# Monokaix/etcd

Measured on AMD Instinct MI355X. Metric: quorum group-evals/sec at 1/2/4/8 MI355X; % HBM peak; speedup vs Go host, higher is better.
Workload: dtype u64; 1 GPU; config2_n5: 64M groups x 5-voter MajorityConfig CommittedIndex+VoteResult (TallyVotes counts into the stats); groups_per_gpu=67108864, global_groups=67108864, voters=5

## Files before the change

etcd_amd/csrc/qe_progress.hpp:

```cpp
#pragma once
#include "qe_tile.hpp"

namespace qe {

constexpr int kRingChunk = 8;

template <bool ACCT>
struct Acct {
  uint64_t b = 0;
  __device__ __forceinline__ void add(bool on, uint32_t bytes) {
    if constexpr (ACCT) b += on ? bytes : 0u;
  }
};
template <bool ACCT>
__device__ __forceinline__ void acct_flush(const Acct<ACCT> &ac, uint64_t *acct) {
  if constexpr (ACCT) {
    uint64_t b = ac.b;
#pragma unroll
    for (int d = 32; d >= 1; d >>= 1) b += __shfl_xor(b, d, 64);
    if ((threadIdx.x & 63) == 0 && acct)
      atomicAdd(reinterpret_cast<unsigned long long *>(acct), static_cast<unsigned long long>(b));
  }
}

// ... 103 lines not shown
  uint32_t added = 0;
  if (x.row) {
    uint32_t fit = 1;
    if (x.me) {
      const uint64_t me = x.me;
      uint32_t q = d >= 4 * me ? 4u : 0u;
      q += d >= (q + 2) * me ? 2u : 0u;
      q += d >= (q + 1) * me ? 1u : 0u;
      fit += q;
    }
    added = x.me ? (lim < fit ? lim : fit) : (lim ? 1u : 0u);
    if (added) {
      if (run.n == 0) {
        run.p = ring_pos(p.start, p.count, x.F);
        run.b = p.next;
      }
      run.n += added;
      const PRun here{0, 0, p.next};
      p.next = run_val(here, added - 1, x.me, x.li) + 1;
      p.count += added;
      ac.add(true, x.eb * added);
    }
  } else {
    while (__builtin_amdgcn_ballot_w64(added < lim && p.next <= x.li)) {
      const bool on = added < lim && p.next <= x.li;
      const PRun here{0, 0, p.next};
      const uint64_t last = run_val(here, 0, x.me, x.li);
      const uint32_t pos = ring_pos(p.start, p.count, x.F);
      ring_add_mem<AUX>(p, x, on, pos, last);
      if (on) {
        if (run.n == 0) {
          run.p = pos;
          run.b = p.next;
        }
        run.n += 1;
        p.next = last + 1;
        p.count += 1;
        added += 1;
      }
      ac.add(on, x.eb);
    }
  }
  if (repl) {
    nmsg = added;
    if (!loop && sei && added < k && p.count < x.F && p.next > x.li) nmsg += k - added;
  }
  if (nmsg) {
    if (x.count_msgs == 0) x.first_index = idx0;
    const uint32_t c = x.count_msgs + (nmsg < 255u ? nmsg : 255u);
    x.count_msgs = c < 255u ? c : 255u;
  }
}

template <bool P>
__device__ __forceinline__ void ring_load_n16(const PSend &x, bool ld, uint32_t rep, uint32_t FP,
                                              uint32_t (&lo)[kRingChunk],
                                              uint32_t (&hi)[kRingChunk], const uint32_t *pre,
                                              uint64_t nx_old) {
  u32x4 a = {0, 0, 0, 0};
  if (pre) {
    a = u32x4{pre[0], pre[1], pre[2], pre[3]};
  } else if (__builtin_amdgcn_ballot_w64(ld)) {
    a = bld128(x.r16, ld ? (threadIdx.x & 63) * 16 : kOOB);
  }
  const uint64_t top = nx_old - 1;
  const uint32_t w4[4] = {a.x, a.y, a.z, a.w};
#pragma unroll
  for (int k = 0; k < kRingChunk; k++) {
    const uint64_t e = top - ((w4[k >> 1] >> (16 * (k & 1))) & 0xFFFFu);
    lo[k] = static_cast<uint32_t>(e);
    hi[k] = static_cast<uint32_t>(e >> 32);
  }
  const bool w = ld && rep_wide(rep);
  if (__builtin_amdgcn_ballot_w64(w)) {
    const u32x4 l0 = bld128(x.rlo, w ? x.lb : kOOB);
    const u32x4 h0 = bld128(x.rhi, w ? x.lb : kOOB);
    u32x4 l1 = {0, 0, 0, 0}, h1 = {0, 0, 0, 0};
    if (FP > 4) {
      l1 = bld128(x.rlo, w ? x.lb + 16 : kOOB);
      h1 = bld128(x.rhi, w ? x.lb + 16 : kOOB);
    }
    if constexpr (P)
      asm volatile("" ::"v"(l0.x), "v"(l0.y), "v"(l0.z), "v"(l0.w), "v"(h0.x), "v"(h0.y),
                   "v"(h0.z), "v"(h0.w), "v"(l1.x), "v"(l1.y), "v"(l1.z), "v"(l1.w), "v"(h1.x),
                   "v"(h1.y), "v"(h1.z), "v"(h1.w));
    if (w) {
      lo[0] = l0.x, lo[1] = l0.y, lo[2] = l0.z, lo[3] = l0.w;
      lo[4] = l1.x, lo[5] = l1.y, lo[6] = l1.z, lo[7] = l1.w;
      hi[0] = h0.x, hi[1] = h0.y, hi[2] = h0.z, hi[3] = h0.w;
      hi[4] = h1.x, hi[5] = h1.y, hi[6] = h1.z, hi[7] = h1.w;
    }
  }
}

template <bool P>
__device__ __forceinline__ void ring_load_row(const PSend &x, bool ld, uint32_t rep, uint32_t FP,
                                              uint32_t (&lo)[kRingChunk],
                                              uint32_t (&hi)[kRingChunk],
                                              const uint32_t *pre = nullptr) {
#pragma unroll
  for (int k = 0; k < kRingChunk; k++) lo[k] = (pre && ld) ? pre[k] : 0u;
  if (!pre && __builtin_amdgcn_ballot_w64(ld)) {
    const u32x4 a = bld128(x.rlo, ld ? x.lb : kOOB);
    lo[0] = a.x, lo[1] = a.y, lo[2] = a.z, lo[3] = a.w;
    if (FP > 4) {
      const u32x4 b = bld128(x.rlo, ld ? x.lb + 16 : kOOB);
      lo[4] = b.x, lo[5] = b.y, lo[6] = b.z, lo[7] = b.w;
    }
  }
  const uint32_t ep = rep_epoch(rep);
#pragma unroll
  for (int k = 0; k < kRingChunk; k++) hi[k] = ep;
  const bool w = ld && rep_wide(rep);
  if (__builtin_amdgcn_ballot_w64(w)) {
    const u32x4 a = bld128(x.rhi, w ? x.lb : kOOB);
    u32x4 b = {0, 0, 0, 0};
    if (FP > 4) b = bld128(x.rhi, w ? x.lb + 16 : kOOB);
    if constexpr (P)
      asm volatile("" ::"v"(a.x), "v"(a.y), "v"(a.z), "v"(a.w), "v"(b.x), "v"(b.y), "v"(b.z),
                   "v"(b.w));
    if (w) hi[0] = a.x, hi[1] = a.y, hi[2] = a.z, hi[3] = a.w;
    if (w) hi[4] = b.x, hi[5] = b.y, hi[6] = b.z, hi[7] = b.w;
  }
}

struct RunLo {
  uint32_t lob, lod, jcap;
};
__device__ __forceinline__ RunLo run_lo(const PRun &r, uint32_t me, uint64_t li) {
  const uint64_t d = li - r.b;
  uint32_t q = 0;
  if (me) {
    const uint64_t m = me;
    q = d >= 4 * m ? 4u : 0u;
    q += d >= (q + 2) * m ? 2u : 0u;
    q += d >= (q + 1) * m ? 1u : 0u;
    q = d >= 8 * m ? 8u : q;
  }
  return RunLo{static_cast<uint32_t>(r.b), static_cast<uint32_t>(d), q};
}
__device__ __forceinline__ uint32_t run_lo_at(const RunLo &L, uint32_t j, uint32_t me) {
  return L.lob + (j < L.jcap ? (j + 1) * me - 1u : L.lod);
}

template <bool P>
// ... 19 lines not shown
    if (!__builtin_amdgcn_ballot_w64(wl && !ok)) {
      const RunLo L1 = run_lo(r1, x.me, x.li), L2 = run_lo(r2, x.me, x.li);
#pragma unroll
      for (int k = 0; k < kRingChunk; k++) {
        if (static_cast<uint32_t>(k) >= x.F) break;
        const uint32_t j1 = static_cast<uint32_t>(k) >= r1.p ? k - r1.p : k + x.F - r1.p;
        const uint32_t j2 = static_cast<uint32_t>(k) >= r2.p ? k - r2.p : k + x.F - r2.p;
        lo[k] = j2 < r2.n ? run_lo_at(L2, j2, x.me) : (j1 < r1.n ? run_lo_at(L1, j1, x.me) : lo[k]);
      }
      if (wl) p.rep = p.count ? QE_PW_EPOCH_BITS(h) : 0u;
      if (P || __builtin_amdgcn_ballot_w64(wl)) {
        bst128(u32x4{lo[0], lo[1], lo[2], lo[3]}, x.rlo, wl ? x.lb : kOOB);
        if (FP > 4) bst128(u32x4{lo[4], lo[5], lo[6], lo[7]}, x.rlo, wl ? x.lb + 16 : kOOB);
      }
      return;
    }
  }
  uint32_t h0 = 0;
  bool seen = false, uni = true;
  const uint32_t st = p.start;
#pragma unroll
  for (int k = 0; k < kRingChunk; k++) {
    if (static_cast<uint32_t>(k) >= x.F) break;
    const uint32_t j1 = static_cast<uint32_t>(k) >= r1.p ? k - r1.p : k + x.F - r1.p;
    const uint32_t j2 = static_cast<uint32_t>(k) >= r2.p ? k - r2.p : k + x.F - r2.p;
    const bool on1 = j1 < r1.n, on2 = j2 < r2.n;
    if (on1 || on2) {
      const uint64_t v = on2 ? run_val(r2, j2, x.me, x.li) : run_val(r1, j1, x.me, x.li);
      lo[k] = static_cast<uint32_t>(v);
      hi[k] = static_cast<uint32_t>(v >> 32);
    }
    const uint32_t rel = static_cast<uint32_t>(k) >= st ? k - st : k + x.F - st;
    if (rel < p.count) {
      uni = uni && (!seen || hi[k] == h0);
      h0 = seen ? h0 : hi[k];
      seen = true;
    }
  }
  const bool wide = seen && (!uni || h0 > QE_RING_EPOCH_MAX);
  if (wl) p.rep = !seen ? 0u : (wide ? QE_PF_RING_WIDE : QE_PW_EPOCH_BITS(h0));
  if (__builtin_amdgcn_ballot_w64(wl)) {
    bst128(u32x4{lo[0], lo[1], lo[2], lo[3]}, x.rlo, wl ? x.lb : kOOB);
    if (FP > 4) bst128(u32x4{lo[4], lo[5], lo[6], lo[7]}, x.rlo, wl ? x.lb + 16 : kOOB);
  }
  const bool wh = wl && wide;
  if (__builtin_amdgcn_ballot_w64(wh)) {
    bst128(u32x4{hi[0], hi[1], hi[2], hi[3]}, x.rhi, wh ? x.lb : kOOB);
    if (FP > 4) bst128(u32x4{hi[4], hi[5], hi[6], hi[7]}, x.rhi, wh ? x.lb + 16 : kOOB);
  }
}

template <bool P>
__device__ __forceinline__ void ring_store_n16(PR &p, const PSend &x, const PRun &r1,
                                               const PRun &r2, bool touched, uint64_t nx_old,
                                               uint32_t FP, uint32_t (&lo)[kRingChunk],
                                               uint32_t (&hi)[kRingChunk]) {
  const bool any = (r1.n | r2.n) != 0;
  const bool wl = touched && p.count > 0 && (any || p.next != nx_old);
  if (!P && !__builtin_amdgcn_ballot_w64(wl)) return;
  const uint64_t top = p.next - 1;
  const uint32_t st = p.start;
  bool fits = true;
  uint32_t o[4] = {0, 0, 0, 0};
#pragma unroll
  for (int k = 0; k < kRingChunk; k++) {
    const uint32_t j1 = static_cast<uint32_t>(k) >= r1.p ? k - r1.p : k + x.F - r1.p;
    const uint32_t j2 = static_cast<uint32_t>(k) >= r2.p ? k - r2.p : k + x.F - r2.p;
    const bool on1 = j1 < r1.n, on2 = j2 < r2.n;
    const uint64_t v = on2 ? run_val(r2, j2, x.me, x.li)
                           : (on1 ? run_val(r1, j1, x.me, x.li) : ent64(hi[k], lo[k]));
    lo[k] = static_cast<uint32_t>(v);
    hi[k] = static_cast<uint32_t>(v >> 32);
    const uint32_t rel = static_cast<uint32_t>(k) >= st ? k - st : k + x.F - st;
    const bool live = static_cast<uint32_t>(k) < x.F && rel < p.count;
    fits = fits && (!live || (v <= top && top - v <= 0xFFFFull));
    o[k >> 1] |= (static_cast<uint32_t>(top - v) & 0xFFFFu) << (16 * (k & 1));
  }
  if (wl) p.rep = fits ? 0u : QE_PF_RING_WIDE;
  if (P || __builtin_amdgcn_ballot_w64(wl))
    bst128(u32x4{o[0], o[1], o[2], o[3]}, x.r16, (wl && fits) ? (threadIdx.x & 63) * 16 : kOOB);
  const bool ww = wl && !fits;
  if (__builtin_amdgcn_ballot_w64(ww)) {
    bst128(u32x4{lo[0], lo[1], lo[2], lo[3]}, x.rlo, ww ? x.lb : kOOB);
    bst128(u32x4{hi[0], hi[1], hi[2], hi[3]}, x.rhi, ww ? x.lb : kOOB);
    if (FP > 4) {
      bst128(u32x4{lo[4], lo[5], lo[6], lo[7]}, x.rlo, ww ? x.lb + 16 : kOOB);
      bst128(u32x4{hi[4], hi[5], hi[6], hi[7]}, x.rhi, ww ? x.lb + 16 : kOOB);
    }
  }
}

__device__ __forceinline__ void ring_append_n16(PR &p, const PSend &x, const PRun &run, bool on,
                                                uint64_t nx_old, uint32_t rep_old, u32x4 raw,
                                                uint32_t FP) {
  const bool wl = on && p.count > 0 && (run.n != 0 || p.next != nx_old);
  if (!__builtin_amdgcn_ballot_w64(wl)) return;
  const uint64_t d64 = p.next - nx_old;
  const uint32_t delta = d64 > 0xFFFFull ? 0x10000u : static_cast<uint32_t>(d64);
  const uint32_t w4[4] = {raw.x, raw.y, raw.z, raw.w};
  const uint32_t st = p.start;
  bool fits = !rep_wide(rep_old);
  uint32_t o[4] = {0, 0, 0, 0};
#pragma unroll
  for (int k = 0; k < kRingChunk; k++) {
    const uint32_t j = static_cast<uint32_t>(k) >= run.p ? k - run.p : k + x.F - run.p;
    const uint32_t rel = static_cast<uint32_t>(k) >= st ? k - st : k + x.F - st;
    const bool live = static_cast<uint32_t>(k) < x.F && rel < p.count;
    uint32_t off;
    if (j < run.n) {
      const uint64_t d = p.next - 1 - run_val(run, j, x.me, x.li);
      off = d > 0xFFFFull ? 0x10000u : static_cast<uint32_t>(d);
    } else {
      off = ((w4[k >> 1] >> (16 * (k & 1))) & 0xFFFFu) + delta;
    }
    fits = fits && (!live || off <= 0xFFFFu);
    o[k >> 1] |= (off & 0xFFFFu) << (16 * (k & 1));
  }
  if (wl && fits) p.rep = 0u;
  bst128(u32x4{o[0], o[1], o[2], o[3]}, x.r16, (wl && fits) ? (threadIdx.x & 63) * 16 : kOOB);
  const bool slow = wl && !fits;
  if (__builtin_amdgcn_ballot_w64(slow)) {
    const bool was_wide = rep_wide(rep_old);
    const uint64_t top_old = nx_old - 1;
    const uint64_t vnew = run.n ? run_val(run, 0, x.me, x.li) : 0;
#pragma unroll 1
    for (uint32_t k = 0; k < x.F; k++) {
      const bool isnew = run.n != 0 && k == run.p;
      const bool wr = slow && (isnew || !was_wide);
      const uint32_t h = k >> 1;
      const uint32_t wd = h == 0 ? raw.x : (h == 1 ? raw.y : (h == 2 ? raw.z : raw.w));
      const uint64_t v = isnew ? vnew : top_old - ((wd >> (16 * (k & 1))) & 0xFFFFu);
      bst32(static_cast<uint32_t>(v), x.rlo, wr ? x.lb + k * 4 : kOOB);
      bst32(static_cast<uint32_t>(v >> 32), x.rhi, wr ? x.lb + k * 4 : kOOB);
    }
    if (slow) p.rep = QE_PF_RING_WIDE;
  }
}

template <bool ACCT>
__device__ __forceinline__ void free_le(PR &p, uint64_t to, uint32_t c_old, uint32_t fr_old,
// ... 72 lines not shown
}
template <typename MT>
__device__ __forceinline__ void ovf_st(uint32_t v, rsrc_t r, uint32_t off) {
  if constexpr (sizeof(MT) == 1) __builtin_amdgcn_raw_buffer_store_b8(static_cast<uint8_t>(v), r, off, 0, 0);
  else __builtin_amdgcn_raw_buffer_store_b16(static_cast<uint16_t>(v), r, off, 0, 0);
}
__device__ __forceinline__ void ovf_fence() { asm volatile("s_waitcnt vmcnt(0)" ::: "memory"); }

struct PB {
  uint64_t mt, ix, nx, hn, lt;
  uint32_t w;
  uint32_t rc;
  uint32_t rl[kRingChunk];
};

struct SlotArgs {
  uint64_t stride;
  uint32_t F, FP;
  uint64_t *match, *next, *pending;
  uint32_t *pw, *ilo, *ihi;
  uint16_t *infl16;
  const uint64_t *mhint, *mlogterm;
  const uint32_t *read_ctx;
  uint8_t *msg_count;
  uint64_t *msg_index;
};

template <bool P>
__device__ __forceinline__ SlotArgs slot_args(const PArgs &a) {
  if constexpr (P) {
    typedef const PArgs __attribute__((address_space(4))) KA;
    KA *ka = (KA *)__builtin_amdgcn_kernarg_segment_ptr();
    asm volatile("" : "+s"(ka));
    return SlotArgs{ka->stride, ka->F, ka->FP, ka->match, ka->next, ka->pending, ka->pw,
                    ka->ilo, ka->ihi, ka->infl16, ka->mhint, ka->mlogterm, ka->read_ctx,
                    ka->msg_count, ka->msg_index};
  } else {
    return SlotArgs{a.stride, a.F, a.FP, a.match, a.next, a.pending, a.pw, a.ilo, a.ihi,
                    a.infl16, a.mhint, a.mlogterm, a.read_ctx, a.msg_count, a.msg_index};
  }
}

template <bool P, bool RD, bool N16, class A>
__device__ __forceinline__ void pb_load(const A &a, uint64_t row, const uint64_t *l_mix,
                                        uint32_t n, uint32_t lane, bool ld, bool rej,
                                        bool has_ix, bool rcl, PB &b) {
  b.mt = l_mix[lane];
  b.ix = has_ix ? l_mix[64 + lane] : 0;
  if constexpr (P) {
    const bool rl = ld;
    if constexpr (N16) {
      const u32x4 x0 = bld128(mk_rsrc(a.infl16 + row * QE_RING16_MAX_F, n * 16), rl ? lane * 16 : kOOB);
      b.rl[0] = x0.x, b.rl[1] = x0.y, b.rl[2] = x0.z, b.rl[3] = x0.w;
      b.rl[4] = b.rl[5] = b.rl[6] = b.rl[7] = 0u;
    } else {
      const rsrc_t rr = mk_rsrc(a.ilo + row * a.FP, n * a.FP * 4);
      const uint32_t lb = lane * a.FP * 4;
      const u32x4 x0 = bld128(rr, rl ? lb : kOOB);
      const u32x4 x1 = bld128(rr, (rl && a.FP > 4) ? lb + 16 : kOOB);
      b.rl[0] = x0.x, b.rl[1] = x0.y, b.rl[2] = x0.z, b.rl[3] = x0.w;
      b.rl[4] = x1.x, b.rl[5] = x1.y, b.rl[6] = x1.z, b.rl[7] = x1.w;
    }
    b.nx = bld64(mk_rsrc(a.next + row, n * 8), ld ? lane * 8 : kOOB);
    b.w = bld32(mk_rsrc(a.pw + row, n * 4), ld ? lane * 4 : kOOB);
    b.hn = bld64(mk_rsrc(a.mhint + row, n * 8), rej ? lane * 8 : kOOB);
    b.lt = bld64(mk_rsrc(a.mlogterm + row, n * 8), rej ? lane * 8 : kOOB);
    if constexpr (RD) b.rc = bld32(opt_rsrc(a.read_ctx, row, n), rcl ? lane * 4 : kOOB);
    else b.rc = 0;
    return;
  }
  if (__builtin_amdgcn_ballot_w64(ld)) {
    b.nx = bld64(mk_rsrc(a.next + row, n * 8), ld ? lane * 8 : kOOB);
    b.w = bld32(mk_rsrc(a.pw + row, n * 4), ld ? lane * 4 : kOOB);
  } else {
    b.nx = 0;
    b.w = 0;
  }
  if (__builtin_amdgcn_ballot_w64(rej)) {
    b.hn = bld64(mk_rsrc(a.mhint + row, n * 8), rej ? lane * 8 : kOOB);
    b.lt = bld64(mk_rsrc(a.mlogterm + row, n * 8), rej ? lane * 8 : kOOB);
  } else {
    b.hn = b.lt = 0;
  }
  if (__builtin_amdgcn_ballot_w64(rcl)) b.rc = bld32(mk_rsrc(a.read_ctx + row, n * 4), rcl ? lane * 4 : kOOB);
  else b.rc = 0;
}

template <bool P>
__device__ __forceinline__ void pb_ready(const PB &b) {
  if constexpr (P) return;
  asm volatile("" ::"v"(b.nx), "v"(b.w), "v"(b.hn), "v"(b.lt), "v"(b.rc));
}

#ifndef QE_PSTEP_WAVES
#define QE_PSTEP_WAVES 3
#endif

template <int S, typename MT, bool MASKED, bool JOINT, int RM, bool ACCT, bool RD,
          int WPB = kBlock / 64, bool P = false, bool N16 = false>
__global__ __attribute__((amdgpu_flat_work_group_size(1, 64 * WPB),
                          amdgpu_waves_per_eu(S <= 9 ? ((N16 && P && !RD && S <= 5) ? 4 : QE_PSTEP_WAVES)
                                                     : 2))) void
k_progress_step(PArgs a) {
  constexpr int CH = kRingChunk;
  constexpr uint32_t kFull = (1u << S) - 1u;
  using QT = typename std::conditional<sizeof(MT) == 1, uint32_t, uint64_t>::type;
  constexpr uint32_t EW = 8 * sizeof(MT);
  constexpr uint32_t kRQ = QE_READ_QUEUE;
  constexpr bool OVF = RD;
  uint32_t n_groups = 0, n_adv = 0, n_viol = 0, n_read = 0;
  uint64_t sum_c = 0, csum = 0;
  Acct<ACCT> ac;
  const uint32_t lane = threadIdx.x & 63;
  const uint64_t wave =
      static_cast<uint64_t>(blockIdx.x) * WPB + __builtin_amdgcn_readfirstlane(threadIdx.x >> 6);
  const uint64_t nwaves = static_cast<uint64_t>(gridDim.x) * WPB;
  const uint64_t ntiles = (a.G + 63) / 64;
  const uint32_t F = a.F;
  static_assert(!P || (S <= 9 && !ACCT), "pipelined form: S <= 9, no accounting");
  const bool row_ring = P || F <= CH;
  constexpr int HD = P ? 2 : 0;
  const uint32_t o8 = lane * 8;
  __shared__ uint64_t l_mix[WPB][S][2][64];
  __shared__ uint64_t l_run[WPB][RM][2][64];
  const uint32_t wv = threadIdx.x >> 6;
  for (uint64_t t = wave; t < ntiles; t += nwaves) {
    const uint64_t g0 = t * 64;
    const uint32_t n = tile_n(a.G, t);
    const bool live = lane < n;
    uint32_t nr = 0;
    const uint32_t mi =
        MASKED ? (ld_mask_r<MT>(mk_rsrc(static_cast<const MT *>(a.inc) + g0, n * sizeof(MT)), lane) &
                  kFull)
               : kFull;
    const uint32_t mo =
        JOINT ? (ld_mask_r<MT>(mk_rsrc(static_cast<const MT *>(a.out) + g0, n * sizeof(MT)), lane) &
                 kFull)
              : 0u;
    const uint32_t trk =
        a.tracked ? (ld_mask_r<MT>(mk_rsrc(static_cast<const MT *>(a.tracked) + g0,
                                           n * sizeof(MT)), lane) & kFull)
                  : kFull;
    const uint32_t self = a.self_slot ? bld8(mk_rsrc(a.self_slot + g0, n), lane) : 0xFFu;
    const uint32_t ltr0 = a.transferee ? bld8(mk_rsrc(a.transferee + g0, n), lane) : 0xFFu;
    uint32_t ltr = ltr0;
    const uint64_t li = bld64(mk_rsrc(a.last_index + g0, n * 8), o8);
    const uint64_t fi = bld64(mk_rsrc(a.first_index + g0, n * 8), o8);
    const uint64_t ts = bld64(mk_rsrc(a.term_start + g0, n * 8), o8);
    const rsrc_t r_commit = mk_rsrc(a.committed + g0, n * 8);
    const uint64_t c0 = bld64(r_commit, o8);
    const uint64_t snap_ld = a.snap_index ? bld64(mk_rsrc(a.snap_index + g0, n * 8), o8) : 0;
    const bool rd = RD && a.read_acks != nullptr;
    uint32_t qh = 0, qn = 0;
    QT q0 = 0;
    if (rd) {
      qn = bld8(mk_rsrc(a.read_count + g0, n), lane);
      qn = qn < a.read_cap ? qn : a.read_cap;
      qh = bld32(mk_rsrc(a.read_head + g0, n * 4), o8 >> 1);
      if constexpr (sizeof(QT) == 4)
        q0 = bld32(mk_rsrc(static_cast<const QT *>(a.read_acks) + g0, n * 4), o8 >> 1);
      else
        q0 = bld64(mk_rsrc(static_cast<const QT *>(a.read_acks) + g0, n * 8), o8);
    }
    const uint32_t dctx = qn ? qh + qn - 1u : 0u;
    const uint32_t qn0 = qn;
    QT q = q0;
    bool qtouch = false;
    uint32_t nrel = 0;
    ac.add(live, (MASKED ? sizeof(MT) : 0) + (JOINT ? sizeof(MT) : 0) +
                     (a.tracked ? sizeof(MT) : 0) + (a.self_slot ? 1 : 0) +
                     (a.transferee ? 1 : 0) + 32 + (a.snap_index ? 8 : 0) + (rd ? 5 : 0) +
                     ((rd && qn0) ? sizeof(QT) : 0));
    uint64_t m0[S];
    uint32_t ty[S];
    uint64_t ix[S];
#pragma unroll
    for (int s = 0; s < S; s++) {
      const uint64_t row = static_cast<uint64_t>(s) * a.stride + g0;
      const bool tr = (trk >> s) & 1u;
      m0[s] = bld64(mk_rsrc(a.match + row, n * 8), o8);
      ty[s] = bld8(mk_rsrc(a.mtype + row, n), tr ? lane : kOOB);
// ... 9 lines not shown
      for (int r = 0; r < RM; r++) {
        const uint64_t rrow = static_cast<uint64_t>(r) * a.stride + g0;
        const uint32_t off = static_cast<uint32_t>(r) < a.R ? o8 : kOOB;
        rr0[r] = bld64(mk_rsrc(a.run_first + rrow, n * 8), off);
        rr1[r] = bld64(mk_rsrc(a.run_term + rrow, n * 8), off);
      }
    }
    uint64_t tys = 0;
    uint32_t msgm = 0, rejm = 0, appm = 0, hbm = 0;
#pragma unroll
    for (int s = 0; s < S; s++) {
      const uint32_t t = ty[s];
      tys |= static_cast<uint64_t>(t <= QE_MSG_TRANSFER_LEADER ? t : 15u) << (4 * s);
      msgm |= (t - 1u <= QE_MSG_TRANSFER_LEADER - 1u ? 1u : 0u) << s;
      rejm |= (t == QE_MSG_APP_RESP_REJECT ? 1u : 0u) << s;
      appm |= (t == QE_MSG_APP_RESP ? 1u : 0u) << s;
      hbm |= (t == QE_MSG_HEARTBEAT_RESP ? 1u : 0u) << s;
    }
    const uint32_t ixm = appm | rejm;
    const uint32_t rcm = (rd && a.read_ctx) ? (hbm & trk) : 0u;
#pragma unroll
    for (int s = 0; s < S; s++) {
      const uint64_t row = static_cast<uint64_t>(s) * a.stride + g0;
      const bool has_ix = ty[s] == QE_MSG_APP_RESP || ty[s] == QE_MSG_APP_RESP_REJECT;
      if constexpr ((HD & 1) == 0) ix[s] = bld64(mk_rsrc(a.mindex + row, n * 8), has_ix ? o8 : kOOB);
      ac.add(has_ix, 8);
      l_mix[wv][s][0][lane] = m0[s];
      l_mix[wv][s][1][lane] = ix[s];
    }
    const bool need_runs = (rejm & trk) != 0;
    if constexpr ((HD & 2) != 0) {
      nr = need_runs ? (rc_all < a.R ? rc_all : a.R) : 0u;
#pragma unroll
      for (int r = 0; r < RM; r++) {
        l_run[wv][r][0][lane] = rr0[r];
        l_run[wv][r][1][lane] = rr1[r];
      }
    } else if (__builtin_amdgcn_ballot_w64(need_runs)) {
      const uint32_t rc = bld8(mk_rsrc(a.run_count + g0, n), need_runs ? lane : kOOB);
      nr = rc < a.R ? rc : a.R;
#pragma unroll
      for (int r = 0; r < RM; r++) {
        const uint64_t rrow = static_cast<uint64_t>(r) * a.stride + g0;
        const uint32_t off = (need_runs && static_cast<uint32_t>(r) < a.R) ? o8 : kOOB;
        l_run[wv][r][0][lane] = bld64(mk_rsrc(a.run_first + rrow, n * 8), off);
        l_run[wv][r][1][lane] = bld64(mk_rsrc(a.run_term + rrow, n * 8), off);
      }
    }
    bool runs_counted = false;
    auto ty_of = [&](uint32_t s) -> uint32_t { return static_cast<uint32_t>(tys >> (4 * s)) & 15u; };
    PB cur;
    constexpr bool PF2 = P && S == 7;
    PB nx1{};
    constexpr bool SKIP = P && S >= 2;
    uint32_t skip = S;
    if constexpr (SKIP) {
      uint32_t um = 0;
#pragma unroll
      for (int s = 0; s < S; s++) {
        const bool may = live && ((((trk & msgm) >> s) & 1u) != 0 ||
                                  (((trk >> s) & 1u) != 0 && self != static_cast<uint32_t>(s)));
        um |= __builtin_amdgcn_ballot_w64(may) ? 0u : (1u << s);
      }
      skip = um ? static_cast<uint32_t>(__builtin_ctz(um)) : static_cast<uint32_t>(S);
    }
    auto after = [&](uint32_t s) -> uint32_t { return s + 1 + (s + 1 == skip ? 1u : 0u); };
    const uint32_t p0 = skip == 0 ? 1u : 0u;
    {
      const bool ld = (((trk & (msgm | (self != p0 ? (1u << p0) : 0u))) >> p0) & 1u) != 0;
      pb_load<P, RD, N16>(a, static_cast<uint64_t>(p0) * a.stride + g0, &l_mix[wv][p0][0][0], n, lane, ld,
                 ((rejm >> p0) & 1u) != 0, ((ixm >> p0) & 1u) != 0, ((rcm >> p0) & 1u) != 0, cur);
    }
    if constexpr (PF2 && S > 2) {
      const uint32_t p1 = after(p0);
      const bool ld = (((trk & (msgm | (self != p1 ? (1u << p1) : 0u))) >> p1) & 1u) != 0;
      pb_load<P, RD, N16>(a, static_cast<uint64_t>(p1) * a.stride + g0, &l_mix[wv][p1][0][0], n, lane, ld,
                 ((rejm >> p1) & 1u) != 0, ((ixm >> p1) & 1u) != 0, ((rcm >> p1) & 1u) != 0, nx1);
    }
    uint64_t c = c0;
    uint64_t cfirst = 0;
    uint32_t bset = 0, upd = 0;
    {
      uint64_t vals[S];
#pragma unroll
      for (int s = 0; s < S; s++) vals[s] = m0[s];
#pragma unroll
      for (int s = 0; s < S; s++) {
        if (ty[s] == QE_MSG_APP_RESP && vals[s] < ix[s]) {
          vals[s] = ix[s];
          upd |= 1u << s;
          const uint64_t mci = mci_of<S, MASKED, JOINT>(vals, mi, mo);
          if (mci > c && mci >= ts && mci <= li) {
            cfirst = bset ? cfirst : mci;
            c = mci;
            bset |= 1u << s;
          }
        }
      }
    }
    pb_ready<P>(cur);
    PSend x;
    x.F = F;
    x.me = a.max_ents;
    x.fi = fi;
    x.li = li;
    x.snap = a.snap_index ? snap_ld : fi - 1;
    x.lb = lane * a.FP * 4;
    x.eb = N16 ? 2u : 4u;
    x.row = row_ring;
    uint32_t sent = 0, snapm = 0, tnow = 0;
    const uint32_t selfb = self < static_cast<uint32_t>(S) ? (1u << self) : 0u;
    const uint32_t tchm = trk & (msgm | (bset != 0 ? (kFull & ~selfb) : 0u));
    const uint32_t ringm = tchm & ((appm & upd) | hbm);
    if constexpr (SKIP) {
      if (skip < static_cast<uint32_t>(S)) {
        const SlotArgs sa = slot_args<P>(a);
        bst8(0u, opt_rsrc(sa.msg_count, static_cast<uint64_t>(skip) * sa.stride + g0, n), lane);
      }
    }
    constexpr int kSlotUnroll = P ? S : 1;
#pragma unroll kSlotUnroll
    for (uint32_t s = 0; s < static_cast<uint32_t>(S); s++) {
      if (SKIP && s == skip) continue;
      const uint32_t s1 = SKIP ? after(s) : s + 1;
      const uint32_t s2 = SKIP ? after(s1) : s + 2;
      const SlotArgs sa = slot_args<P>(a);
      const uint64_t row = static_cast<uint64_t>(s) * sa.stride + g0;
      const uint32_t tt = ty_of(s);
      const bool touched = ((tchm >> s) & 1u) != 0;
      PB nxt{};
      if constexpr (PF2) {
        if (s2 < static_cast<uint32_t>(S)) {
          pb_load<P, RD, N16>(sa, static_cast<uint64_t>(s2) * sa.stride + g0, &l_mix[wv][s2][0][0], n, lane,
                     ((tchm >> s2) & 1u) != 0, ((rejm >> s2) & 1u) != 0, ((ixm >> s2) & 1u) != 0,
                     ((rcm >> s2) & 1u) != 0, nxt);
        }
        cur.mt = l_mix[wv][s][0][lane];
        cur.ix = ((ixm >> s) & 1u) ? l_mix[wv][s][1][lane] : 0;
      } else if (s1 < static_cast<uint32_t>(S)) {
        pb_load<P, RD, N16>(sa, static_cast<uint64_t>(s1) * sa.stride + g0, &l_mix[wv][s1][0][0], n, lane,
                   ((tchm >> s1) & 1u) != 0, ((rejm >> s1) & 1u) != 0, ((ixm >> s1) & 1u) != 0,
                   ((rcm >> s1) & 1u) != 0, nxt);
      }
      if (!P && !__builtin_amdgcn_ballot_w64(touched)) {
        pb_ready<P>(nxt);
        if (sa.msg_count) bst8(0u, mk_rsrc(sa.msg_count + row, n), lane);
        ac.add(live && sa.msg_count, 1);
        if (s1 < static_cast<uint32_t>(S)) cur = nxt;
        continue;
      }
      ac.add(touched, 12);
      ac.add(touched && tt == QE_MSG_APP_RESP_REJECT, 16);
      ac.add(touched && ((rcm >> s) & 1u), 4);
      PR p;
      p.match = cur.mt;
      p.next = cur.nx;
      pr_unpack(p, cur.w);
      p.reset = 0;
      const uint32_t rep0 = p.rep;
      const uint64_t nx_old = cur.nx;
      const bool need_pd = touched && p.state == QE_PR_SNAPSHOT;
      uint64_t pd0 = 0;
      if (__builtin_amdgcn_ballot_w64(need_pd)) {
        pd0 = bld64(mk_rsrc(sa.pending + row, n * 8), need_pd ? o8 : kOOB);
        if constexpr (P) asm volatile("" ::"v"(pd0));
        ac.add(need_pd, 8);
      }
      p.pending = pd0;
      {
        const uint64_t rb = (static_cast<uint64_t>(s) * sa.stride + g0) * sa.FP;
        x.rlo = mk_rsrc(sa.ilo + rb, n * sa.FP * 4);
        x.rhi = mk_rsrc(sa.ihi + rb, n * sa.FP * 4);
        if constexpr (N16) x.r16 = mk_rsrc(sa.infl16 + row * QE_RING16_MAX_F, n * 16);
      }
      const bool up = (upd >> s) & 1u;
      const uint32_t c_old = p.count;
      uint32_t rlo[kRingChunk], rhi[kRingChunk];
      uint32_t npre = 0;
      if (N16) {
        ring_load_n16<P>(x, touched && c_old > 0, rep0, sa.FP, rlo, rhi, P ? cur.rl : nullptr,
                         nx_old);
      } else if (row_ring) {
        ring_load_row<P>(x, touched && c_old > 0, rep0, sa.FP, rlo, rhi, P ? cur.rl : nullptr);
      } else {
#pragma unroll
        for (int k = 0; k < CH; k++) rlo[k] = rhi[k] = 0;
        const bool scan = ((ringm >> s) & 1u) != 0 && p.state == QE_PR_REPLICATE;
        npre = scan ? (c_old < CH ? c_old : CH) : 0u;
        if (__builtin_amdgcn_ballot_w64(npre > 0)) {
#pragma unroll
          for (int k = 0; k < CH; k++) {
            uint32_t pos = p.start + k;
            if (pos >= F) pos -= F;
            if (pos >= F) pos = 0;
            const uint64_t v = ring_get_mem(x, rep0, static_cast<uint32_t>(k) < npre, pos);
            rlo[k] = static_cast<uint32_t>(v);
            rhi[k] = static_cast<uint32_t>(v >> 32);
          }
        }
      }
      x.count_msgs = 0;
      x.first_index = 0;
      x.snapped = false;
      PRun r1{0, 0, 0}, r2{0, 0, 0};
      const bool bcast_target = touched && s != self;
      const uint32_t below = (1u << s) - 1u;
      const uint32_t k1 = bcast_target ? popc(bset & below) : 0u;
      const uint32_t k3 = bcast_target ? popc(bset & ~below & ~(1u << s)) : 0u;
      uint32_t k2 = 0;
      bool lp = false;
      pb_ready<P>(nxt);
      if (__builtin_amdgcn_ballot_w64(k1 > 0)) send_burst<ACCT>(p, true, k1, x, r1, ac);
      uint32_t rel = 0;
      bool ovf_hit = false;
      if (touched) {
        if (tt == QE_MSG_APP_RESP_REJECT) {
          p.recent_active = 1;
          uint64_t probe = cur.hn;
          if (cur.lt > 0) {
            uint64_t rf[RM], rt[RM];
#pragma unroll
            for (int r = 0; r < RM; r++) {
              rf[r] = l_run[wv][r][0][lane];
              rt[r] = l_run[wv][r][1][lane];
            }
            probe = find_conflict_by_term<RM>(rf, rt, nr, li, probe, cur.lt);
            ac.add(!runs_counted, 1 + 16 * nr);
            runs_counted = true;
          }
          bool decr;
          if (p.state == QE_PR_REPLICATE) {
            decr = cur.ix > p.match;
            if (decr) p.next = p.match + 1;
          } else {
            decr = (p.next - 1 == cur.ix);
            if (decr) {
              const uint64_t m = cur.ix < probe + 1 ? cur.ix : probe + 1;
              p.next = m > 1 ? m : 1;
              p.probe_sent = 0;
            }
          }
          if (decr && p.state == QE_PR_REPLICATE) pr_become_probe(p);
          k2 = decr ? 1u : 0u;
        } else if (tt == QE_MSG_APP_RESP) {
          p.recent_active = 1;
          const uint64_t idx = cur.ix;
          n_viol += (idx > li);
          const bool old_paused = pr_paused(p, F);
          if (up) {
            p.match = idx;
            p.probe_sent = 0;
          }
          if (p.next < idx + 1) p.next = idx + 1;
          if (up) {
            if (p.state == QE_PR_PROBE) {
              pr_become_replicate(p);
            } else if (p.state == QE_PR_SNAPSHOT && p.match >= p.pending) {
              pr_become_probe(p);
              pr_become_replicate(p);
            } else if (p.state == QE_PR_REPLICATE) {
              const uint32_t fo = row_ring ? row_prefix_le(rlo, rhi, F, p.start, c_old, idx)
                                           : mem_prefix_le(rlo, rhi, npre, p.start, c_old, idx, rep0, x);
              free_le<ACCT>(p, idx, c_old, fo, r1, x, ac);
            }
            k2 = ((bset >> s) & 1u) ? (s != self ? 1u : 0u) : (old_paused ? 1u : 0u);
            lp = true;
            if (s == ltr && p.match == li) tnow |= 1u << s;
          }
        } else if (tt == QE_MSG_HEARTBEAT_RESP) {
          p.recent_active = 1;
          p.probe_sent = 0;
          if (p.state == QE_PR_REPLICATE && p.count == F) {
            uint64_t first;
            if (c_old == 0) first = run_val(r1, 0, x.me, li);
            else if (row_ring) first = row_at(rlo, rhi, p.start < F ? p.start : 0u);
            else first = ent64(rhi[0], rlo[0]);
            const uint32_t fo = row_ring ? row_prefix_le(rlo, rhi, F, p.start, c_old, first)
                                         : mem_prefix_le(rlo, rhi, npre, p.start, c_old, first, rep0, x);
            free_le<ACCT>(p, first, c_old, fo, r1, x, ac);
          }
          k2 = p.match < li ? 1u : 0u;
          if (rd) {
            const uint32_t cx = sa.read_ctx ? cur.rc : dctx;
            const uint32_t j = cx - qh;
            if (cx != 0 && j < kRQ && j < qn) {
              q |= static_cast<QT>(1u << s) << (EW * j);
              qtouch = true;
              const uint32_t e = static_cast<uint32_t>(q >> (EW * j)) & kFull;
              if (joint_vote(mi, mo, e, e) == kVoteWon) rel = j + 1;
            }
            ovf_hit = OVF && cx != 0 && j >= kRQ && j < qn;
          }
        } else if (tt == QE_MSG_SNAP_STATUS || tt == QE_MSG_SNAP_STATUS_REJECT) {
          if (p.state == QE_PR_SNAPSHOT) {
            if (tt == QE_MSG_SNAP_STATUS_REJECT) p.pending = 0;
            pr_become_probe(p);
            p.probe_sent = 1;
          }
        } else if (tt == QE_MSG_UNREACHABLE) {
          if (p.state == QE_PR_REPLICATE) pr_become_probe(p);
        } else if (tt == QE_MSG_TRANSFER_LEADER) {
          if ((((mi | mo) >> s) & 1u) != 0) {
            bool go = true;
            if (ltr < static_cast<uint32_t>(S)) {
              if (ltr == s) go = false;
              else ltr = 0xFFu;
            }
            if (s == self) go = false;
            if (go) {
              ltr = s;
              if (p.match == li) tnow |= 1u << s;
              else k2 = 1;
            }
          }
        }
      }
      if constexpr (RD) {
        if (OVF && __builtin_amdgcn_ballot_w64(ovf_hit)) {
          ovf_fence();
          const uint32_t ovf_ctx = sa.read_ctx ? cur.rc : dctx;
          const rsrc_t r_ovf = ovf_rsrc<MT>(a, g0, n);
          const uint32_t off = ovf_hit ? ovf_off(a, lane, ovf_ctx, sizeof(MT)) : kOOB;
          const uint32_t e = ovf_ld<MT>(r_ovf, off) | (1u << s);
          const bool won = ovf_hit && joint_vote(mi, mo, e & kFull, e & kFull) == kVoteWon;
          ovf_st<MT>(e, r_ovf, (ovf_hit && !won) ? off : kOOB);
          rel = won ? ovf_ctx - qh + 1u : rel;
          ac.add(ovf_hit, sizeof(MT));
          ac.add(ovf_hit && !won, sizeof(MT));
        }
        if (__builtin_amdgcn_ballot_w64(rel != 0)) {
          const uint32_t qn_old = qn;
          if (rel != 0) {
            q = rel >= kRQ ? static_cast<QT>(0) : static_cast<QT>(q >> (EW * rel));
            qh += rel;
            qn -= rel;
            nrel += rel;
            qtouch = true;
          }
          if (OVF && __builtin_amdgcn_ballot_w64(rel != 0 && qn_old > kRQ)) {
            ovf_fence();
            const rsrc_t r_ovf = ovf_rsrc<MT>(a, g0, n);
#pragma unroll 1
            for (uint32_t pp = 0; pp < kRQ; pp++) {
              const bool on = rel != 0 && qn_old > kRQ && pp < qn && pp + rel >= kRQ;
              const uint32_t e = ovf_ld<MT>(r_ovf, on ? ovf_off(a, lane, qh + pp, sizeof(MT)) : kOOB);
              if (on) q |= static_cast<QT>(e) << (EW * pp);
              ac.add(on, sizeof(MT));
            }
          }
        }
      }
      const uint32_t km = lp ? kLoop : k2 + k3;
      if (__builtin_amdgcn_ballot_w64(km > 0)) send_burst<ACCT>(p, lp ? k2 != 0 : true, km, x, r2, ac);
      if (__builtin_amdgcn_ballot_w64(lp && k3 > 0)) send_burst<ACCT>(p, true, lp ? k3 : 0u, x, r2, ac);
      if constexpr (N16) ring_store_n16<P>(p, x, r1, r2, touched, nx_old, sa.FP, rlo, rhi);
      else if (row_ring) ring_store_row<P>(p, x, r1, r2, touched, rep0, c_old, sa.FP, rlo, rhi);
      const uint32_t nw = pr_pack(p);
      const bool tw = touched;
      const bool wm = tw && up, wn = tw && p.next != cur.nx;
      const bool wp = tw && p.pending != pd0;
      const bool ww = tw && nw != cur.w;
      const bool fm = wm, fn = wn, fw = ww;
      const bool wc = touched && ((nw ^ cur.w) & ~QE_PW_RING_MASK) != 0;
      constexpr bool PIPE = P;
      if (PIPE || __builtin_amdgcn_ballot_w64(wm))
        bst64(p.match, mk_rsrc(sa.match + row, n * 8), fm ? o8 : kOOB);
      if (PIPE || __builtin_amdgcn_ballot_w64(wn))
        bst64(p.next, mk_rsrc(sa.next + row, n * 8), fn ? o8 : kOOB);
      if (__builtin_amdgcn_ballot_w64(wp))
        bst64(p.pending, mk_rsrc(sa.pending + row, n * 8), wp ? o8 : kOOB);
      if (PIPE || __builtin_amdgcn_ballot_w64(ww))
        bst32(nw, mk_rsrc(sa.pw + row, n * 4), fw ? lane * 4 : kOOB);
      if (PIPE) {
        bst8(x.count_msgs, opt_rsrc(sa.msg_count, row, n), lane);
        bst64(x.first_index, opt_rsrc(sa.msg_index, row, n), x.count_msgs ? o8 : kOOB);
      } else {
        if (sa.msg_count) bst8(x.count_msgs, mk_rsrc(sa.msg_count + row, n), lane);
        if (sa.msg_index && __builtin_amdgcn_ballot_w64(x.count_msgs != 0))
          bst64(x.first_index, mk_rsrc(sa.msg_index + row, n * 8), x.count_msgs ? o8 : kOOB);
      }
      ac.add(wm, 8);
      ac.add(wn, 8);
      ac.add(wp, 8);
      ac.add(wc, 4);
      ac.add(live && sa.msg_count, 1);
      ac.add(x.count_msgs && sa.msg_index, 8);
      sent |= x.count_msgs ? (1u << s) : 0u;
      snapm |= x.snapped ? (1u << s) : 0u;
      if (s1 < static_cast<uint32_t>(S)) {
        if constexpr (PF2) {
          cur = nx1;
          nx1 = nxt;
        } else {
          cur = nxt;
        }
      }
    }
    const uint32_t bc = popc(bset);
    bst64(c, r_commit, c != c0 ? o8 : kOOB);
    if (a.sent) bst_mask<MT>(sent, opt_rsrc(static_cast<const MT *>(a.sent), g0, n), lane);
    if (a.snap) bst_mask<MT>(snapm, opt_rsrc(static_cast<const MT *>(a.snap), g0, n), lane);
    if (a.tnow) bst_mask<MT>(tnow, opt_rsrc(static_cast<const MT *>(a.tnow), g0, n), lane);
    if (a.bcast) bst8(bc, opt_rsrc(static_cast<const uint8_t *>(a.bcast), g0, n), lane);
    if (rd) {
      const QT canon = qn >= kRQ ? q : static_cast<QT>(q & ((static_cast<QT>(1) << (EW * qn)) - 1u));
      const bool wq = qtouch && canon != q0, wr = nrel != 0;
      if (__builtin_amdgcn_ballot_w64(wq)) {
        if constexpr (sizeof(QT) == 4)
          bst32(canon, mk_rsrc(static_cast<QT *>(a.read_acks) + g0, n * 4), wq ? o8 >> 1 : kOOB);
        else
          bst64(canon, mk_rsrc(static_cast<QT *>(a.read_acks) + g0, n * 8), wq ? o8 : kOOB);
      }
      if (__builtin_amdgcn_ballot_w64(wr)) {
        bst32(qh, mk_rsrc(a.read_head + g0, n * 4), wr ? o8 >> 1 : kOOB);
        bst8(qn, mk_rsrc(a.read_count + g0, n), wr ? lane : kOOB);
      }
      ac.add(wq, sizeof(QT));
      ac.add(wr, 5);
    }
    if (a.read_released) bst8(nrel, opt_rsrc(a.read_released, g0, n), lane);
    ac.add(live && a.read_released, 1);
    const bool tc = c != c0 && !(c0 >= ts && c0 <= li);
    if (a.term_commit) bst8(tc ? 1u : 0u, opt_rsrc(a.term_commit, g0, n), lane);
    if (a.term_commit_index && __builtin_amdgcn_ballot_w64(tc))
      bst64(cfirst, mk_rsrc(a.term_commit_index + g0, n * 8), tc ? o8 : kOOB);
    ac.add(live && a.term_commit, 1);
    ac.add(tc && a.term_commit_index, 8);
    const bool wt = a.transferee && ltr != ltr0;
    if (__builtin_amdgcn_ballot_w64(wt)) bst8(ltr, mk_rsrc(a.transferee + g0, n), wt ? lane : kOOB);
    ac.add(wt, 1);
    ac.add(live && c != c0, 8);
    ac.add(live && a.sent, sizeof(MT));
    ac.add(live && a.snap, sizeof(MT));
    ac.add(live && a.tnow, sizeof(MT));
    ac.add(live && a.bcast, 1);
    if (live) {
      const uint64_t gh = (a.goff + g0 + lane) * kPhi;
      n_groups += 1;
      sum_c += c;
      n_adv += (c != c0);
      n_read += nrel;
      csum += mix64(gh ^ c ^ (static_cast<uint64_t>(bc) << 62)) +
                     mix64(gh ^ (static_cast<uint64_t>(sent) << 40) ^ kSentSalt) +
                     (nrel ? mix64(gh ^ kReadSalt ^ (static_cast<uint64_t>(nrel) << 56)) : 0ull) +
                     (tc ? mix64(gh ^ kTermSalt ^ cfirst) : 0ull) +
                     (ltr != ltr0 ? mix64(gh ^ kTransferSalt ^ ltr) : 0ull);
    }
  }
  if (a.stats) {
    const int idx[P_N] = {QE_STAT_GROUPS, QE_STAT_COMMIT_SUM, QE_STAT_COMMIT_ADVANCED,
                          QE_STAT_INVARIANT_VIOLATIONS, QE_STAT_READ_RELEASED,
                          QE_STAT_CHECKSUM};
    uint64_t cnt[P_N];
    cnt[P_GROUPS] = n_groups;
    cnt[P_SUM] = sum_c;
    cnt[P_ADV] = n_adv;
    cnt[P_VIOL] = n_viol;
    cnt[P_READ] = n_read;
    cnt[P_CSUM] = csum;
    block_stats_add<P_N, 64 * WPB>(cnt, idx, a.stats);
  }
  acct_flush<ACCT>(ac, a.acct);
}

constexpr int kSendTPW = 8;

template <int S>
struct SendSet {
  uint64_t fi, li, sn;
  uint64_t nx[S];
  uint32_t pw[S];
};

template <int S>
__device__ __forceinline__ void ps_issue(const PArgs &a, uint64_t t, uint32_t lane, uint32_t w,
                                         SendSet<S> &x) {
  const uint64_t g0 = t * 64;
  const uint32_t n = tile_n(a.G, t);
  const uint32_t o8 = lane * 8, o4 = lane * 4;
  x.fi = bld64<kNT>(mk_rsrc(a.first_index + g0, n * 8), w ? o8 : kOOB);
  x.li = bld64<kNT>(mk_rsrc(a.last_index + g0, n * 8), w ? o8 : kOOB);
  x.sn = a.snap_index ? bld64<kNT>(mk_rsrc(a.snap_index + g0, n * 8), w ? o8 : kOOB) : 0;
#pragma unroll
  for (int s = 0; s < S; s++) {
    const uint64_t row = static_cast<uint64_t>(s) * a.stride + g0;
    x.nx[s] = bld64<kNT>(mk_rsrc(a.next + row, n * 8), bit_off(w, s, o8));
    x.pw[s] = bld32<kNT>(mk_rsrc(a.pw + row, n * 4), bit_off(w, s, o4));
  }
}

// ... 933 lines not shown
```

Before: 125.4 billion group-evals/s.

## Keep n16 inflight ring packed in registers instead of expanding to 64-bit rows

Replaces the n16 ring load, which expanded the packed 16-bit offsets into eight 64-bit lo/hi entries, with a path that keeps only the four packed words. Prefix-free scans and the ring store work directly on those offsets, and the wide ring is read per entry from memory only when some lane needs it. It also moves the cur.mt/ix LDS reads later in pipelined variants and pins the group-id base into a scalar register. The aim is to cut VGPR pressure and ALU work on the common narrow path. The cost is more complex control flow and slow serial per-entry loads on the wide fallback.

```diff
diff --git a/etcd_amd/csrc/qe_progress.hpp b/etcd_amd/csrc/qe_progress.hpp
--- a/etcd_amd/csrc/qe_progress.hpp
+++ b/etcd_amd/csrc/qe_progress.hpp
@@ -179,45 +179,52 @@
   }
 }
 
-template <bool P>
-__device__ __forceinline__ void ring_load_n16(const PSend &x, bool ld, uint32_t rep, uint32_t FP,
-                                              uint32_t (&lo)[kRingChunk],
-                                              uint32_t (&hi)[kRingChunk], const uint32_t *pre,
-                                              uint64_t nx_old) {
-  u32x4 a = {0, 0, 0, 0};
-  if (pre) {
-    a = u32x4{pre[0], pre[1], pre[2], pre[3]};
-  } else if (__builtin_amdgcn_ballot_w64(ld)) {
-    a = bld128(x.r16, ld ? (threadIdx.x & 63) * 16 : kOOB);
-  }
+__device__ __forceinline__ uint32_t n16_off(const uint32_t (&w)[4], int k) {
+  return (w[k >> 1] >> (16 * (k & 1))) & 0xFFFFu;
+}
+__device__ __forceinline__ uint32_t n16_off_at(const uint32_t (&w)[4], uint32_t pos) {
+  uint32_t v = 0;
+#pragma unroll
+  for (int h = 0; h < 4; h++)
+    v |= w[h] & (0u - static_cast<uint32_t>((pos >> 1) == static_cast<uint32_t>(h)));
+  return (v >> (16 * (pos & 1u))) & 0xFFFFu;
+}
+__device__ __forceinline__ uint32_t n16_prefix_le(const uint32_t (&w)[4], uint32_t F,
+                                                  uint32_t start, uint32_t c_old,
+                                                  uint64_t nx_old, uint64_t to) {
   const uint64_t top = nx_old - 1;
-  const uint32_t w4[4] = {a.x, a.y, a.z, a.w};
-#pragma unroll
-  for (int k = 0; k < kRingChunk; k++) {
-    const uint64_t e = top - ((w4[k >> 1] >> (16 * (k & 1))) & 0xFFFFu);
-    lo[k] = static_cast<uint32_t>(e);
-    hi[k] = static_cast<uint32_t>(e >> 32);
-  }
-  const bool w = ld && rep_wide(rep);
-  if (__builtin_amdgcn_ballot_w64(w)) {
-    const u32x4 l0 = bld128(x.rlo, w ? x.lb : kOOB);
-    const u32x4 h0 = bld128(x.rhi, w ? x.lb : kOOB);
-    u32x4 l1 = {0, 0, 0, 0}, h1 = {0, 0, 0, 0};
-    if (FP > 4) {
-      l1 = bld128(x.rlo, w ? x.lb + 16 : kOOB);
-      h1 = bld128(x.rhi, w ? x.lb + 16 : kOOB);
-    }
-    if constexpr (P)
-      asm volatile("" ::"v"(l0.x), "v"(l0.y), "v"(l0.z), "v"(l0.w), "v"(h0.x), "v"(h0.y),
-                   "v"(h0.z), "v"(h0.w), "v"(l1.x), "v"(l1.y), "v"(l1.z), "v"(l1.w), "v"(h1.x),
-                   "v"(h1.y), "v"(h1.z), "v"(h1.w));
-    if (w) {
-      lo[0] = l0.x, lo[1] = l0.y, lo[2] = l0.z, lo[3] = l0.w;
-      lo[4] = l1.x, lo[5] = l1.y, lo[6] = l1.z, lo[7] = l1.w;
-      hi[0] = h0.x, hi[1] = h0.y, hi[2] = h0.z, hi[3] = h0.w;
-      hi[4] = h1.x, hi[5] = h1.y, hi[6] = h1.z, hi[7] = h1.w;
-    }
-  }
+  const uint64_t gap = top - to;
+  const uint32_t thr = to >= top ? 0u : (gap > 0xFFFFull ? 0x10000u : static_cast<uint32_t>(gap));
+  const uint32_t cap = top > 0xFFFFull ? 0xFFFFu : static_cast<uint32_t>(top);
+  const bool some = thr <= cap;
+  const uint32_t t = some ? thr : 0x10000u, span = some ? cap - thr : 0u;
+  uint32_t pm = 0;
+#pragma unroll
+  for (int k = 0; k < kRingChunk; k++) pm |= (n16_off(w, k) - t) <= span ? (1u << k) : 0u;
+  const uint32_t full = (1u << F) - 1u;
+  pm &= full;
+  const uint32_t st = start < F ? start : 0u;
+  const uint32_t rk = ((pm >> st) | (pm << (F - st))) & full;
+  const uint32_t run = __builtin_ctz(~rk);
+  return run < c_old ? run : c_old;
+}
+__device__ __forceinline__ uint32_t wide_prefix_le(const PSend &x, bool on, uint32_t start,
+                                                   uint32_t c_old, bool first_one, uint64_t &to) {
+  uint32_t pos = start < x.F ? start : 0u;
+  uint32_t fr = 0;
+  bool go = on;
+#pragma unroll 1
+  for (uint32_t r = 0; r < x.F; r++) {
+    go = go && r < c_old;
+    if (!__builtin_amdgcn_ballot_w64(go)) break;
+    const uint32_t off = go ? x.lb + pos * 4 : kOOB;
+    const uint64_t v = ent64(bld32(x.rhi, off), bld32(x.rlo, off));
+    if (go && first_one && r == 0) to = v;
+    go = go && v <= to;
+    fr += go ? 1u : 0u;
+    if (++pos >= x.F) pos = 0;
+  }
+  return fr;
 }
 
 template <bool P>
@@ -343,40 +350,90 @@
 
 template <bool P>
 __device__ __forceinline__ void ring_store_n16(PR &p, const PSend &x, const PRun &r1,
-                                               const PRun &r2, bool touched, uint64_t nx_old,
-                                               uint32_t FP, uint32_t (&lo)[kRingChunk],
-                                               uint32_t (&hi)[kRingChunk]) {
+                                               const PRun &r2, bool touched, bool wa,
+                                               uint64_t nx_old, uint32_t FP,
+                                               const uint32_t (&w)[4]) {
   const bool any = (r1.n | r2.n) != 0;
   const bool wl = touched && p.count > 0 && (any || p.next != nx_old);
   if (!P && !__builtin_amdgcn_ballot_w64(wl)) return;
   const uint64_t top = p.next - 1;
+  const uint32_t cap = top > 0xFFFFull ? 0xFFFFu : static_cast<uint32_t>(top);
+  const uint64_t d64 = p.next - nx_old;
+  const uint32_t dl = d64 + 0x10000ull <= 0x20000ull
+                          ? static_cast<uint32_t>(d64)
+                          : (0x20000u | (static_cast<uint32_t>(d64) & 0xFFFFu));
   const uint32_t st = p.start;
-  bool fits = true;
+  auto run_at = [&](uint32_t k, bool &on) -> uint64_t {
+    const uint32_t j1 = k >= r1.p ? k - r1.p : k + x.F - r1.p;
+    const uint32_t j2 = k >= r2.p ? k - r2.p : k + x.F - r2.p;
+    const bool on2 = j2 < r2.n;
+    on = on2 || j1 < r1.n;
+    const PRun r{0, 0, on2 ? r2.b : r1.b};
+    return run_val(r, on2 ? j2 : j1, x.me, x.li);
+  };
+  auto live_at = [&](uint32_t k) -> bool {
+    const uint32_t rel = k >= st ? k - st : k + x.F - st;
+    return k < x.F && rel < p.count;
+  };
+  uint32_t lm;
+  {
+    const uint32_t c = p.count < x.F ? p.count : x.F;
+    const uint32_t m = (1u << c) - 1u;
+    const bool wrap = st < x.F;
+    const uint32_t sh = wrap ? st : (st - x.F < 31u ? st - x.F : 31u);
+    lm = ((m << sh) | (wrap ? m >> (x.F - st) : 0u)) & ((1u << x.F) - 1u);
+  }
+  uint32_t mx = 0;
   uint32_t o[4] = {0, 0, 0, 0};
 #pragma unroll
   for (int k = 0; k < kRingChunk; k++) {
-    const uint32_t j1 = static_cast<uint32_t>(k) >= r1.p ? k - r1.p : k + x.F - r1.p;
-    const uint32_t j2 = static_cast<uint32_t>(k) >= r2.p ? k - r2.p : k + x.F - r2.p;
-    const bool on1 = j1 < r1.n, on2 = j2 < r2.n;
-    const uint64_t v = on2 ? run_val(r2, j2, x.me, x.li)
-                           : (on1 ? run_val(r1, j1, x.me, x.li) : ent64(hi[k], lo[k]));
-    lo[k] = static_cast<uint32_t>(v);
-    hi[k] = static_cast<uint32_t>(v >> 32);
-    const uint32_t rel = static_cast<uint32_t>(k) >= st ? k - st : k + x.F - st;
-    const bool live = static_cast<uint32_t>(k) < x.F && rel < p.count;
-    fits = fits && (!live || (v <= top && top - v <= 0xFFFFull));
-    o[k >> 1] |= (static_cast<uint32_t>(top - v) & 0xFFFFu) << (16 * (k & 1));
+    bool on;
+    const uint64_t d = top - run_at(k, on);
+    const uint32_t dr = d > 0xFFFFull ? (0x10000u | (static_cast<uint32_t>(d) & 0xFFFFu))
+                                      : static_cast<uint32_t>(d);
+    const uint32_t off = on ? dr : n16_off(w, k) + dl;
+    const uint32_t offl = off & (0u - ((lm >> k) & 1u));
+    mx = mx > offl ? mx : offl;
+    o[k >> 1] |= (off & 0xFFFFu) << (16 * (k & 1));
+  }
+  bool fits = mx <= cap;
+  if (__builtin_amdgcn_ballot_w64(wl && wa)) {
+    fits = fits && !wa;
+    bool f2 = true;
+#pragma unroll 1
+    for (uint32_t k = 0; k < kRingChunk; k++) {
+      bool on;
+      const uint64_t rv = run_at(k, on);
+      const uint32_t a = (wl && wa && k < FP) ? x.lb + k * 4 : kOOB;
+      const uint64_t ev = ent64(bld32(x.rhi, a), bld32(x.rlo, a));
+      const uint64_t v = on ? rv : ev;
+      f2 = f2 && (!live_at(k) || (v <= top && top - v <= 0xFFFFull));
+      if (wa) {
+        o[0] = (o[0] >> 16) | (o[1] << 16);
+        o[1] = (o[1] >> 16) | (o[2] << 16);
+        o[2] = (o[2] >> 16) | (o[3] << 16);
+        o[3] = (o[3] >> 16) | (static_cast<uint32_t>(top - v) << 16);
+      }
+    }
+    fits = fits || (wa && f2);
   }
   if (wl) p.rep = fits ? 0u : QE_PF_RING_WIDE;
   if (P || __builtin_amdgcn_ballot_w64(wl))
     bst128(u32x4{o[0], o[1], o[2], o[3]}, x.r16, (wl && fits) ? (threadIdx.x & 63) * 16 : kOOB);
   const bool ww = wl && !fits;
   if (__builtin_amdgcn_ballot_w64(ww)) {
-    bst128(u32x4{lo[0], lo[1], lo[2], lo[3]}, x.rlo, ww ? x.lb : kOOB);
-    bst128(u32x4{hi[0], hi[1], hi[2], hi[3]}, x.rhi, ww ? x.lb : kOOB);
-    if (FP > 4) {
-      bst128(u32x4{lo[4], lo[5], lo[6], lo[7]}, x.rlo, ww ? x.lb + 16 : kOOB);
-      bst128(u32x4{hi[4], hi[5], hi[6], hi[7]}, x.rhi, ww ? x.lb + 16 : kOOB);
+    const uint64_t top_old = nx_old - 1;
+    uint64_t wlo = ent64(w[1], w[0]), whi = ent64(w[3], w[2]);
+#pragma unroll 1
+    for (uint32_t k = 0; k < FP; k++) {
+      bool on;
+      const uint64_t rv = run_at(k, on);
+      const uint64_t v = on ? rv : top_old - (wlo & 0xFFFFull);
+      wlo = (wlo >> 16) | (whi << 48);
+      whi >>= 16;
+      const bool wr = ww && (on || !wa);
+      bst32(static_cast<uint32_t>(v), x.rlo, wr ? x.lb + k * 4 : kOOB);
+      bst32(static_cast<uint32_t>(v >> 32), x.rhi, wr ? x.lb + k * 4 : kOOB);
     }
   }
 }
@@ -555,7 +612,6 @@
     if constexpr (N16) {
       const u32x4 x0 = bld128(mk_rsrc(a.infl16 + row * QE_RING16_MAX_F, n * 16), rl ? lane * 16 : kOOB);
       b.rl[0] = x0.x, b.rl[1] = x0.y, b.rl[2] = x0.z, b.rl[3] = x0.w;
-      b.rl[4] = b.rl[5] = b.rl[6] = b.rl[7] = 0u;
     } else {
       const rsrc_t rr = mk_rsrc(a.ilo + row * a.FP, n * a.FP * 4);
       const uint32_t lb = lane * a.FP * 4;
@@ -629,7 +685,8 @@
   const uint32_t wv = threadIdx.x >> 6;
   for (uint64_t t = wave; t < ntiles; t += nwaves) {
     const uint64_t g0 = t * 64;
-    const uint32_t n = tile_n(a.G, t);
+    const uint64_t rem = a.G - g0;
+    const uint32_t n = rem < 64 ? static_cast<uint32_t>(rem) : 64u;
     const bool live = lane < n;
     uint32_t nr = 0;
     const uint32_t mi =
@@ -745,6 +802,7 @@
     PB cur;
     constexpr bool PF2 = P && S == 7;
     PB nx1{};
+    constexpr bool LATE = PF2 || (P && N16 && !RD && S <= 5);
     constexpr bool SKIP = P && S >= 2;
     uint32_t skip = S;
     if constexpr (SKIP) {
@@ -828,12 +886,14 @@
                      ((tchm >> s2) & 1u) != 0, ((rejm >> s2) & 1u) != 0, ((ixm >> s2) & 1u) != 0,
                      ((rcm >> s2) & 1u) != 0, nxt);
         }
-        cur.mt = l_mix[wv][s][0][lane];
-        cur.ix = ((ixm >> s) & 1u) ? l_mix[wv][s][1][lane] : 0;
       } else if (s1 < static_cast<uint32_t>(S)) {
         pb_load<P, RD, N16>(sa, static_cast<uint64_t>(s1) * sa.stride + g0, &l_mix[wv][s1][0][0], n, lane,
                    ((tchm >> s1) & 1u) != 0, ((rejm >> s1) & 1u) != 0, ((ixm >> s1) & 1u) != 0,
                    ((rcm >> s1) & 1u) != 0, nxt);
+      }
+      if constexpr (LATE) {
+        cur.mt = l_mix[wv][s][0][lane];
+        cur.ix = ((ixm >> s) & 1u) ? l_mix[wv][s][1][lane] : 0;
       }
       if (!P && !__builtin_amdgcn_ballot_w64(touched)) {
         pb_ready<P>(nxt);
@@ -870,9 +930,15 @@
       const uint32_t c_old = p.count;
       uint32_t rlo[kRingChunk], rhi[kRingChunk];
       uint32_t npre = 0;
-      if (N16) {
-        ring_load_n16<P>(x, touched && c_old > 0, rep0, sa.FP, rlo, rhi, P ? cur.rl : nullptr,
-                         nx_old);
+      uint32_t rw[4] = {0, 0, 0, 0};
+      const bool wa = N16 && touched && c_old > 0 && rep_wide(rep0);
+      if constexpr (N16) {
+        if constexpr (P) {
+          rw[0] = cur.rl[0], rw[1] = cur.rl[1], rw[2] = cur.rl[2], rw[3] = cur.rl[3];
+        } else if (__builtin_amdgcn_ballot_w64(touched && c_old > 0)) {
+          const u32x4 q = bld128(x.r16, (touched && c_old > 0) ? lane * 16 : kOOB);
+          rw[0] = q.x, rw[1] = q.y, rw[2] = q.z, rw[3] = q.w;
+        }
       } else if (row_ring) {
         ring_load_row<P>(x, touched && c_old > 0, rep0, sa.FP, rlo, rhi, P ? cur.rl : nullptr);
       } else {
@@ -952,8 +1018,18 @@
               pr_become_probe(p);
               pr_become_replicate(p);
             } else if (p.state == QE_PR_REPLICATE) {
-              const uint32_t fo = row_ring ? row_prefix_le(rlo, rhi, F, p.start, c_old, idx)
-                                           : mem_prefix_le(rlo, rhi, npre, p.start, c_old, idx, rep0, x);
+              uint32_t fo;
+              if constexpr (N16) {
+                fo = n16_prefix_le(rw, F, p.start, c_old, nx_old, idx);
+                if (__builtin_amdgcn_ballot_w64(wa)) {
+                  uint64_t to = idx;
+                  const uint32_t fw = wide_prefix_le(x, wa, p.start, c_old, false, to);
+                  fo = wa ? fw : fo;
+                }
+              } else {
+                fo = row_ring ? row_prefix_le(rlo, rhi, F, p.start, c_old, idx)
+                              : mem_prefix_le(rlo, rhi, npre, p.start, c_old, idx, rep0, x);
+              }
               free_le<ACCT>(p, idx, c_old, fo, r1, x, ac);
             }
             k2 = ((bset >> s) & 1u) ? (s != self ? 1u : 0u) : (old_paused ? 1u : 0u);
@@ -966,10 +1042,22 @@
           if (p.state == QE_PR_REPLICATE && p.count == F) {
             uint64_t first;
             if (c_old == 0) first = run_val(r1, 0, x.me, li);
+            else if (N16) first = nx_old - 1 - n16_off_at(rw, p.start < F ? p.start : 0u);
             else if (row_ring) first = row_at(rlo, rhi, p.start < F ? p.start : 0u);
             else first = ent64(rhi[0], rlo[0]);
-            const uint32_t fo = row_ring ? row_prefix_le(rlo, rhi, F, p.start, c_old, first)
-                                         : mem_prefix_le(rlo, rhi, npre, p.start, c_old, first, rep0, x);
+            uint32_t fo;
+            if constexpr (N16) {
+              fo = n16_prefix_le(rw, F, p.start, c_old, nx_old, first);
+              if (__builtin_amdgcn_ballot_w64(wa)) {
+                uint64_t to = first;
+                const uint32_t fw = wide_prefix_le(x, wa, p.start, c_old, true, to);
+                first = wa ? to : first;
+                fo = wa ? fw : fo;
+              }
+            } else {
+              fo = row_ring ? row_prefix_le(rlo, rhi, F, p.start, c_old, first)
+                            : mem_prefix_le(rlo, rhi, npre, p.start, c_old, first, rep0, x);
+            }
             free_le<ACCT>(p, first, c_old, fo, r1, x, ac);
           }
           k2 = p.match < li ? 1u : 0u;
@@ -1046,7 +1134,7 @@
       const uint32_t km = lp ? kLoop : k2 + k3;
       if (__builtin_amdgcn_ballot_w64(km > 0)) send_burst<ACCT>(p, lp ? k2 != 0 : true, km, x, r2, ac);
       if (__builtin_amdgcn_ballot_w64(lp && k3 > 0)) send_burst<ACCT>(p, true, lp ? k3 : 0u, x, r2, ac);
-      if constexpr (N16) ring_store_n16<P>(p, x, r1, r2, touched, nx_old, sa.FP, rlo, rhi);
+      if constexpr (N16) ring_store_n16<P>(p, x, r1, r2, touched, wa, nx_old, sa.FP, rw);
       else if (row_ring) ring_store_row<P>(p, x, r1, r2, touched, rep0, c_old, sa.FP, rlo, rhi);
       const uint32_t nw = pr_pack(p);
       const bool tw = touched;
@@ -1128,7 +1216,9 @@
     ac.add(live && a.tnow, sizeof(MT));
     ac.add(live && a.bcast, 1);
     if (live) {
-      const uint64_t gh = (a.goff + g0 + lane) * kPhi;
+      uint64_t gid0 = a.goff + g0;
+      asm volatile("" : "+s"(gid0));
+      const uint64_t gh = (gid0 + lane) * kPhi;
       n_groups += 1;
       sum_c += c;
       n_adv += (c != c0);
```

Result: slower. 120.6 billion group-evals/s (-3.8%).
